# silverlight6/Ultrasound_Modeling

Hardware: AMD Instinct MI355X
Metric: segmentation training images/sec at 256x256 (higher is better)
Workload: dtype bf16

## Files before the change

### include/usseg.h

```cpp
#ifndef USSEG_H
#define USSEG_H

#include <stddef.h>
#include <stdint.h>

#ifdef __cplusplus
extern "C" {
#endif

typedef void* usseg_stream_t;

typedef enum UssegStatus {
  USSEG_OK = 0,
  USSEG_ERR_BAD_ARG = -1,
  USSEG_ERR_UNSUPPORTED = -2,
  USSEG_ERR_LAUNCH = -3
} UssegStatus;

typedef enum UssegAct { USSEG_ACT_NONE = 0, USSEG_ACT_LRELU = 1, USSEG_ACT_RELU = 2, USSEG_ACT_ELU = 3, USSEG_ACT_GELU = 4 } UssegAct;

enum {
  USSEG_OUT_F32 = 1,
  USSEG_ACCUMULATE = 2
};
// ... 49 lines not shown
int usseg_tconv2d_wgrad_mapped(const UssegConvDesc* d, const void* x, const void* dy, const UssegWgradDst* dst, float* ws,
                               int64_t ws_floats, usseg_stream_t stream);

typedef struct UssegWgradJob {
  UssegConvDesc desc;
  const void* x;
  const void* dy;
  float* dw;
  const UssegWgradDst* dst;
} UssegWgradJob;
int usseg_conv2d_wgrad_multi(int32_t njobs, const UssegWgradJob* jobs, float* ws, int64_t ws_floats, usseg_stream_t stream);

int usseg_defer_begin(usseg_stream_t stream, float* reduce_ws, int64_t reduce_floats, float* wgrad_ws, int64_t wgrad_floats);
int usseg_defer_flush(usseg_stream_t stream);
int usseg_defer_end(usseg_stream_t stream);

typedef struct UssegConvJob {
  UssegConvDesc desc;
  const void* x;
  const void* wp;
  const float* bias;
  const void* residual;
  int32_t ldr;
  int32_t reserved;
  void* y;
  const float* scale;
} UssegConvJob;
int usseg_conv2d_fwd_multi(int32_t njobs, const UssegConvJob* jobs, usseg_stream_t stream);
int usseg_conv2d_dgrad_multi(int32_t njobs, const UssegConvJob* jobs, usseg_stream_t stream);

// ... 377 lines not shown
```

### ultrasound_modeling_amd/_lib.py

```python
from __future__ import annotations

import ctypes as C
import os

import torch
from . import knobs

_HERE = os.path.dirname(os.path.abspath(__file__))
LIB_PATH = knobs.get("USSEG_LIB") or os.path.join(_HERE, "libusseg_hip.so")

c_i32, c_i64, c_f32, c_vp = C.c_int32, C.c_int64, C.c_float, C.c_void_p


class UssegError(RuntimeError):
    pass


class ConvDesc(C.Structure):
    _fields_ = [("B", c_i32), ("H", c_i32), ("W", c_i32), ("Cin", c_i32), ("Cout", c_i32), ("ldx", c_i32),
                ("ldy", c_i32), ("ksize", c_i32), ("dilation", c_i32), ("act", c_i32), ("alpha", c_f32),
                ("flags", c_i32)]


class ConvJob(C.Structure):
# ... 208 lines not shown
    "usseg_scale_f32": (C.c_int, [c_vp, c_i64, c_vp, c_f32, c_vp]),
    "usseg_sched_advance": (C.c_int, [c_vp, c_vp, c_vp, c_vp, c_f32, c_f32, c_vp]),
    "usseg_sumsq_sched_advance": (C.c_int, [c_vp, c_i64, c_vp, c_vp, c_vp, c_vp, c_vp, c_f32, c_f32, c_vp]),
    "usseg_adamw_step": (C.c_int, [c_vp, c_vp, c_vp, c_vp, c_i64, c_vp, c_f32, c_vp, c_vp, c_vp, c_f32, c_f32, c_f32, c_vp]),
    "usseg_gemm_nt_batched": (C.c_int, [P(GemmDesc), c_vp, c_vp, c_vp, c_vp]),
    "usseg_gemm_tn_batched": (C.c_int, [P(GemmDesc), c_vp, c_vp, c_vp, c_vp]),
    "usseg_flash_attn_fwd": (C.c_int, [P(FlashDesc), c_vp, c_vp, c_vp, c_vp, c_vp, c_vp, c_vp]),
    "usseg_flash_attn_bwd": (C.c_int, [P(FlashDesc), c_vp, c_vp, c_vp, c_vp, c_vp, c_vp, c_vp, c_vp, c_vp, c_vp, c_vp, c_vp]),
    "usseg_softmax_rows_fwd": (C.c_int, [c_vp, c_i64, c_i32, c_f32, c_vp, c_vp, c_vp]),
    "usseg_softmax_rows_bwd": (C.c_int, [c_vp, c_vp, c_i64, c_i32, c_f32, c_vp, c_vp]),
    "usseg_transpose_batched": (C.c_int, [c_vp, c_i32, c_i32, c_i32, c_i32, c_i32, c_i64, c_i64, c_vp, c_vp]),
    "usseg_cast_f32_to_bf16_batched": (C.c_int, [c_vp, c_i32, c_i32, c_i32, c_i32, c_vp, c_i32, c_i64, c_i64, c_vp]),
    "usseg_defer_begin": (C.c_int, [c_vp, c_vp, c_i64, c_vp, c_i64]),
    "usseg_defer_flush": (C.c_int, [c_vp]),
    "usseg_defer_end": (C.c_int, [c_vp]),
    "usseg_prof_enable": (C.c_int, [c_i32, c_i32]),
    "usseg_prof_read": (C.c_int, [c_i32, P(C.c_double), P(c_i64)]),
    "usseg_prof_disable": (C.c_int, []),
    "usseg_prep_cycle_stats": (C.c_int, [c_vp, c_i32, c_i32, c_i32, c_vp, c_vp, c_vp]),
    "usseg_prep_label": (C.c_int, [c_vp, c_i32, c_i32, c_vp, c_vp, c_i32, c_i32, c_i32, c_vp, c_vp, c_vp, c_vp]),
    "usseg_prep_label_thick": (C.c_int, [c_vp, c_i32, c_i32, c_vp, c_i32, c_i32, c_i32, c_vp, c_vp, c_vp]),
    "usseg_prep_assemble": (C.c_int, [c_vp, c_vp, c_i32, c_i32, c_i32, c_vp, c_i32, c_i32, c_i32, c_vp, c_vp, c_i32, c_vp, c_vp]),
    "usseg_select_ranks_f64": (C.c_int, [c_vp, c_i32, c_i64, P(c_i32), c_i32, c_vp, c_vp, c_vp]),
    "usseg_prep_aug_ws_doubles": (c_i64, [c_i32, c_i32, c_i32, c_i32, c_i32]),
    "usseg_prep_aug": (C.c_int, [P(PrepAugDesc), c_vp, c_vp, c_vp, c_vp, c_vp, c_i64, c_vp, c_vp, c_vp]),
    "usseg_cone_index": (C.c_int, [c_vp, c_vp, c_i32, c_i32, C.c_double, C.c_double, C.c_double, c_i32, c_i32, c_vp, c_vp]),
    "usseg_cone_range": (C.c_int, [c_vp, c_i32, c_i32, c_vp, c_vp, c_vp]),
    "usseg_cone_render": (C.c_int, [c_vp, c_i32, c_i32, c_i32, c_vp, c_vp, c_vp, c_vp, c_i32, c_i32, c_i32, P(C.c_double), c_vp, c_vp, c_vp,
                                    c_vp]),
}
# ... 26 lines not shown
```

### ultrasound_modeling_amd/csrc/common.h

```cpp
#pragma once
#include <hip/hip_runtime.h>
#include <stdint.h>
#include <stdio.h>
#include <stdlib.h>
#include "../../include/usseg.h"
#include "knobs.h"

typedef unsigned short bf16_t;
typedef __attribute__((ext_vector_type(8))) __bf16 bf16x8_t;
typedef __attribute__((ext_vector_type(4))) float f32x4_t;
typedef __attribute__((ext_vector_type(4))) short s16x4_t;

__device__ __forceinline__ float fdiv_rcp(int d) { return 0.5f * __builtin_amdgcn_rcpf((float)d); }
__device__ __forceinline__ int fdiv(int n, float r) {
  float x;
  asm("v_mul_f32_e32 %0, %1, %2" : "=v"(x) : "v"((float)(2 * n + 1)), "v"(r));
  return (int)x;
}
__device__ __forceinline__ void fdivmod(int n, int d, float r, int& q, int& rem) {
  q = fdiv(n, r);
  rem = n - __mul24(q, d);
}

__device__ __forceinline__ float fdiv_rcp1(int d) { return __builtin_amdgcn_rcpf((float)d); }
// ... 392 lines not shown
  UssegTapMask mask = {};
};
static inline WgHaloGeom wgrad_halo_geom(const UssegConvDesc& d, const void* x, const void* dy, float* out, const WgMap& map,
                                         const UssegTapMask& mask = {}) {
  WgHaloGeom g = {(const bf16_t*)x, (const bf16_t*)dy, out, map, d.B, d.H, d.W, d.dilation, d.Cin, d.Cout, d.ldx, d.ldy};
  g.mask = mask;
  return g;
}
int usseg_try_launch_wgrad_halo(const WgHaloGeom* g, int njobs, float* ws, int64_t ws_floats, hipStream_t s);
int conv2d_wgrad_impl(const UssegConvDesc* d, const void* x, const void* dy, float* dw, const UssegWgradDst* dst, float* ws, int64_t ws_floats,
                      const UssegTapMask& mask, usseg_stream_t stream);

float* usseg_defer_reduce_ws(hipStream_t s, float* caller_ws, int64_t need);
void usseg_defer_reduce_ws_n(hipStream_t s, float* caller_ws, const int64_t* need, int n, float** out);
float* usseg_defer_wgrad_ws(hipStream_t s, float* caller_ws, int64_t caller_floats, int64_t* avail);
void usseg_launch_wgrad_finish(const float* ws, int splits, int64_t slab_floats, float* out, const WgMap& map, int Ma, int Nb, hipStream_t s);

int usseg_try_launch_tconv_wgrad_halo(const bf16_t* x, const bf16_t* dy, const WgMap& map, int B, int H, int W, int Cin, int Cout, int ldx,
                                      int lddy, int k, float* ws, int64_t ws_floats, hipStream_t s);

static inline int64_t cdiv64(int64_t a, int64_t b) { return (a + b - 1) / b; }
```

### ultrasound_modeling_amd/csrc/defer.hip

```cpp
#include <vector>
#include "common.h"

struct RJob {
  const float* ws;
  float *d0, *d1, *d2;
  int32_t groups, nb, K, Cp, C, nblocks;
  float scale;
  int32_t overwrite;
};
struct RBatch {
  int32_t njobs, pad;
  int32_t start[60];
  RJob job[59];
};
static_assert(sizeof(RBatch) <= 4096, "RBatch must fit the kernel-argument segment");

__device__ __forceinline__ void reduce_finish_body(const RJob& q, int bx, int nbx) {
  __shared__ float s_part[16][17];
  const int total = q.groups * q.K * q.C;
  const int o = threadIdx.x & 15, sl = threadIdx.x >> 4;
  for (int base = bx * 16; base < total; base += nbx * 16) {
    const int i = base + o;
    float s = 0.f;
    int c = 0, k = 0, g = 0;
// ... 146 lines not shown
    RBatch b = {};
    int total = 0;
    while (i < c.rj.size() && b.njobs < 59 && !rjob_shares_dst(b, c.rj[i])) {
      b.job[b.njobs] = c.rj[i++];
      b.start[b.njobs] = total;
      total += b.job[b.njobs].nblocks;
      ++b.njobs;
    }
    b.start[b.njobs] = total;
    hipLaunchKernelGGL(reduce_finish_batched_kernel, dim3(total), dim3(256), 0, c.s, b);
  }
  c.rj.clear();
  c.rused = 0;
}
static void flush_wgrad(DeferCtx& c) {
  size_t i = 0;
  while (i < c.wj.size()) {
    WBatch b = {};
    int total = 0;
    while (i < c.wj.size() && b.njobs < 14 && !wjob_shares_dst(b, c.wj[i])) {
      b.job[b.njobs] = c.wj[i++];
      b.start[b.njobs] = total;
      total += b.job[b.njobs].gx;
      ++b.njobs;
    }
    b.start[b.njobs] = total;
    const int slot = usseg_prof_start(2, c.s);
    hipLaunchKernelGGL(wgrad_finish_batched_kernel, dim3(total), dim3(256), 0, c.s, b);
    usseg_prof_stop(2, slot, c.s);
  }
// ... 32 lines not shown
  if (c && c->rws && ws >= c->rws && ws < c->rws + c->rcap) {
    c->rj.push_back(q);
    return;
  }
  hipLaunchKernelGGL(reduce_finish_kernel, dim3(grid), dim3(256), 0, s, q);
}

float* usseg_defer_wgrad_ws(hipStream_t s, float* caller_ws, int64_t caller_floats, int64_t* avail) {
  DeferCtx* c = find_ctx(s);
  if (!c || !c->wws) { *avail = caller_floats; return caller_ws; }
  if (c->wcap - c->wused < c->wcap / 4 && !c->wj.empty()) flush_wgrad(*c);
  *avail = c->wcap - c->wused;
  return c->wws + c->wused;
}

void usseg_launch_wgrad_finish(const float* ws, int splits, int64_t slab_floats, float* out, const WgMap& map, int Ma, int Nb, hipStream_t s) {
  WJob q = {};
  q.ws = ws; q.out = out; q.n4 = slab_floats / 4; q.splits = splits; q.Ma = Ma; q.Nb = Nb; q.map = map;
  int sl_log2 = 2;
  while (sl_log2 < 6 && (q.n4 + (256 >> sl_log2) - 1) / (256 >> sl_log2) < 256 && splits >= (2 << (sl_log2 + 2))) sl_log2 += 2;
  const int O = 256 >> sl_log2;
  int gx = (int)((q.n4 + O - 1) / O);
  if (gx > 2048) gx = 2048;
  q.gx = gx; q.sl_log2 = sl_log2;
  DeferCtx* c = find_ctx(s);
  if (c && c->wws && ws >= c->wws && ws < c->wws + c->wcap) {
    c->wused = (ws - c->wws) + (((int64_t)splits * slab_floats + 63) & ~(int64_t)63);
    c->wj.push_back(q);
    return;
  }
  hipLaunchKernelGGL(wgrad_finish_kernel, dim3(gx), dim3(256), 0, s, q);
}

extern "C" int usseg_defer_begin(usseg_stream_t stream, float* reduce_ws, int64_t reduce_floats, float* wgrad_ws, int64_t wgrad_floats) {
  USSEG_CHECK_ARG((!reduce_ws || reduce_floats > 0) && (!wgrad_ws || wgrad_floats > 0), "defer_begin: bad workspace sizes");
  hipStream_t s = (hipStream_t)stream;
  DeferCtx* c = find_ctx(s);
  if (c) { flush_reduce(*c); flush_wgrad(*c); }
  else { g_ctx.push_back(DeferCtx()); c = &g_ctx.back(); c->s = s; }
  c->rws = reduce_ws; c->rcap = reduce_ws ? reduce_floats : 0; c->rused = 0;
  c->wws = wgrad_ws; c->wcap = wgrad_ws ? wgrad_floats : 0; c->wused = 0;
  return USSEG_OK;
// ... 18 lines not shown
```

### ultrasound_modeling_amd/csrc/knobs.h

```cpp
#pragma once
#include <stdint.h>
#include <stdlib.h>

#define USSEG_KNOBS(X)                                                                                                                  \
                                                                                                                      \
  X(K_BIG,                "USSEG_BIG",                INT,     1,     ONCE,     "0: conv_big and the streaming conv take no launch")        \
  X(K_BIG_PX,             "USSEG_BIG_PX",             INT,     0,     ONCE,     "conv_big: force the pixel tile (128 / 256; 0: planner)")   \
  X(K_BIG_NT,             "USSEG_BIG_NT",             INT,     0,     ONCE,     "conv_big: force the channel tile (1 / 2 / 4 x 16; 0: planner)") \
  X(K_BIG_MIN_WG,         "USSEG_BIG_MIN_WG",         INT,     128,   ONCE,     "conv_big: smallest launch it takes, in workgroups")        \
  X(K_BIG_WG_TILE,        "USSEG_BIG_WG_TILE",        INT,     512,   ONCE,     "conv_big: narrow the channel tile below this many workgroups") \
  X(K_BIG_MIN_CIN,        "USSEG_BIG_MIN_CIN",        INT,     33,    ONCE,     "conv_big: fewest input channels of a pass it takes")       \
  X(K_BIG_STAGES,         "USSEG_BIG_STAGES",         INT,     0,     ONCE,     "conv_big LDS stages: 0 by launch size, 1 / 2 forced")      \
  X(K_BIG_W8,             "USSEG_BIG_W8",             INT,     1,     PER_CALL, "256-pixel tile on eight waves: 0 never, 1 planner, 2 forced") \
  X(K_BIG_W8_MIN,         "USSEG_BIG_W8_MIN",         INT,     128,   ONCE,     "fewest workgroups left for the eight-wave tile")           \
  X(K_STREAM,             "USSEG_STREAM",             INT,     1,     ONCE,     "0: the streaming conv takes no launch")                    \
  X(K_STREAM_PX,          "USSEG_STREAM_PX",          INT,     0,     ONCE,     "streaming conv: force the pixel tile (128 / 256; 0: planner)") \
  X(K_STREAM_MIN_STEPS,   "USSEG_STREAM_MIN_STEPS",   INT,     1,     PER_CALL, "streaming conv: fewest K steps per workgroup it takes")    \
  X(K_STREAM_WGX,         "USSEG_STREAM_WGX",         INT,     0,     PER_CALL, "streaming conv: force grid.x (>= 8, rounded down to a multiple of 8)") \
  X(K_STREAM_OCC,         "USSEG_STREAM_OCC",         INT,     0,     ONCE,     "streaming conv: cap on workgroups per CU (0: by LDS)")     \
  X(K_STREAM_RES,         "USSEG_STREAM_RES",         INT,     1,     ONCE,     "0: passes with a residual do not stream")                  \
  X(K_STREAM_MULTI,       "USSEG_STREAM_MULTI",       INT,     1,     ONCE,     "0: multi-job launches do not stream")                      \
  X(K_STREAM_MERGE,       "USSEG_STREAM_MERGE",       INT,     1,     PER_CALL, "streaming jobs of one plan in one launch (0: a launch per job)") \
                                                                                                     \
  X(K_NO_HALO,            "USSEG_NO_HALO",            PRESENT, 0,     ONCE,     "the halo-tile conv and weight-gradient kernels take no launch") \
// ... 7 lines not shown
  X(K_IGEMM_DMA_BATCHED,  "USSEG_IGEMM_DMA_BATCHED",  INT,     1,     ONCE,     "0: batched GEMMs stay on the register-staged igemm")       \
  X(K_IGEMM_XCD,          "USSEG_IGEMM_XCD",          INT,     1,     ONCE,     "XCD-aware item order: 0 off, 1 activation-heavy launches, 2 all") \
  X(K_IGEMM_PERSIST,      "USSEG_IGEMM_PERSIST",      INT,     1,     ONCE,     "0: never the persistent LDS-DMA igemm")                    \
  X(K_IGEMM_STAGES8,      "USSEG_IGEMM_STAGES8",      INT,     4,     ONCE,     "ring depth of sparse long-K 128-channel launches (2: off, 3, 4)") \
  X(K_IGEMM_STAGES8_WG,   "USSEG_IGEMM_STAGES8_WG",   INT,     256,   ONCE,     "largest launch, in workgroups, that gets the deeper ring") \
                                                                                                         \
  X(K_WGRAD_DMA,          "USSEG_WGRAD_DMA",          INT,     1,     ONCE,     "0: never the LDS-DMA per-tap weight gradient / batched TN GEMM") \
  X(K_WGRAD_TM,           "USSEG_WGRAD_TM",           INT,     0,     ONCE,     "per-tap wgrad: force the tile (1: 64x64, 2: 128x128; 0: planner)") \
  X(K_WGD_TARGET,         "USSEG_WGD_TARGET",         INT,     512,   ONCE,     "per-tap wgrad: workgroups the split-K aims for")           \
  X(K_WGD_CAP,            "USSEG_WGD_CAP",            INT,     4,     ONCE,     "per-tap wgrad: slab traffic cap, in multiples of the operand bytes") \
  X(K_WG_QUANT,           "USSEG_WG_QUANT",           INT,     1,     ONCE,     "0: no wave-quantisation search of the split count (both wgrad kernels)") \
  X(K_WGRAD_DEBUG,        "USSEG_WGRAD_DEBUG",        PRESENT, 0,     ONCE,     "print every weight-gradient plan to stderr")               \
  X(K_WGRAD_POW2,         "USSEG_WGRAD_POW2",         INT,     1,     ONCE,     "0: no shift decode of power-of-two grids")                 \
  X(K_WGRAD_XCD,          "USSEG_WGRAD_XCD",          INT,     1,     ONCE,     "0: no XCD-aware item order in the per-tap wgrad")          \
  X(K_WG_TARGET,          "USSEG_WG_TARGET",          INT,     256,   ONCE,     "halo wgrad: workgroups the split-K aims for")              \
  X(K_SLAB_CAP,           "USSEG_SLAB_CAP",           INT,     2,     ONCE,     "halo wgrad: slab traffic cap, in multiples of the operand bytes") \
  X(K_WGHALO_XCD,         "USSEG_WGHALO_XCD",         INT,     1,     ONCE,     "0: no XCD-aware item order in the halo wgrad")             \
  X(K_WGRAD_PF,           "USSEG_WGRAD_PF",           INT,     1,     ONCE,     "0: halo wgrad without the register prefetch")              \
  X(K_WGRAD_8W,           "USSEG_WGRAD_8W",           INT,     1,     ONCE,     "0: the 64x64 halo wgrad tile on four waves, not eight")    \
  X(K_TCONV_HALO,         "USSEG_TCONV_HALO",         INT,     0,     PER_CALL, "1: transposed-conv wgrad as four parity-class halo jobs")  \
                                                                                                                      \
  X(K_CARD_BWD_G,         "USSEG_CARD_BWD_G",         INT,     0,     ONCE,     "fused cardinal backward: force the workgroup pairs (0: one resident wave)") \
  X(K_LN_TILE,            "USSEG_LN_TILE",            INT,     1,     ONCE,     "0: never the tile LayerNorm backward")                     \
  X(K_LN_PAIR,            "USSEG_LN_PAIR",            INT,     1,     ONCE,     "0: never the paired LayerNorm backward launch")            \
  X(K_LN_TILE_MIN,        "USSEG_LN_TILE_MIN",        INT,     32768, ONCE,     "fewest pixels for the tile / paired LayerNorm backward")   \
                                                                                     \
  X(K_FLASH_TILE,         "USSEG_FLASH_TILE",         INT,     -1,    ONCE,     "fused attention tiling 0 / 1 / 2 (-1: by problem size)")   \
  X(K_WINATTN_MFMA,       "USSEG_WINATTN_MFMA",       INT,     1,     ONCE,     "0: window attention without the MFMA kernels")             \
  X(K_LOSS_PPT,           "USSEG_LOSS_PPT",           INT,     4,     ONCE,     "softmax + loss kernel: pixels per thread")

// ... 26 lines not shown
```

### ultrasound_modeling_amd/csrc/wgrad_halo.hip

```cpp
#include "common.h"

struct WgHaloParams {
  const bf16_t* x;
  const bf16_t* dy;
  float* out;
  float* ws;
  int32_t B, H, W, d, Hl, Wl, PH, PW, NV;
  int32_t tiles_x, tiles_per_v, npatches, ngroups, groups_per_block;
  int32_t ldx, lddy, Ma, Nb, ntiles_n;
  int32_t mask_ch;
  uint16_t tapmask[4];
  int32_t xvd, xvH, xvW, xva, xvb;
  int32_t yvd, yvH, yvW, yva, yvb;
};

struct WgHaloMulti {
  WgHaloParams job[4];
  int32_t xcd_remap;
};

template <int WVM, int WM, int WN, bool PF, int NTG, bool MASKED>
__global__ __launch_bounds__(256 * NTG, NTG == 1 ? 2 : 1) void wgrad_halo_kernel(const WgHaloMulti P) {
  constexpr int NTHR = 256 * NTG, TPG = NTG == 1 ? 9 : 5;
  int bx = blockIdx.x, by = blockIdx.y, bz = blockIdx.z;
  if (P.xcd_remap) {
    const int gx = gridDim.x, gy = gridDim.y, gz = gridDim.z, total = gx * gy * gz;
    const int L = bx + gx * (by + gy * bz);
    const int c = L & 7, q = total >> 3, r = total & 7;
    const int item = c * q + (c < r ? c : r) + (L >> 3);
    const int u = __builtin_amdgcn_readfirstlane(fdiv(item, fdiv_rcp(gy)));
    by = item - u * gy;
    bx = __builtin_amdgcn_readfirstlane(fdiv(u, fdiv_rcp(gz)));
    bz = u - bx * gz;
  }
  const WgHaloParams& p = P.job[bz];
  constexpr int MAXHP = 288;
  constexpr int WVN = 4 / WVM;
  constexpr int BMc = 16 * WM * WVM, BNc = 16 * WN * WVN;
  constexpr int XS = BMc + 16, YS = BNc == 16 ? 48 : BNc + 16;
  constexpr int XCH = BMc / 8, YCH = BNc / 8;
  constexpr int X_IT = (MAXHP * XCH + NTHR - 1) / NTHR, Y_IT = (128 * YCH + NTHR - 1) / NTHR;
  __shared__ __attribute__((aligned(16))) bf16_t lds_x[MAXHP * XS];
  __shared__ __attribute__((aligned(16))) bf16_t lds_y[128 * YS];
  constexpr int TB = NTHR / 8;
  __shared__ __attribute__((aligned(16))) int s_tab[TB][8][8];

  const int tid = threadIdx.x, lane = tid & 63, wv = (tid >> 6) & 3, tg = tid >> 8;
  const int t0 = tg * TPG;
  const int HW2 = p.PW + 2, HPP = (p.PH + 2) * HW2, NHP = p.NV * HPP;
  const int rps = 16 / p.PW, spp = (p.PH * p.PW) >> 4;
// ... 248 lines not shown
        if (m >= p.Ma || n >= p.Nb) continue;
        float* q = dst + ((int64_t)t * p.Ma + m) * p.Nb + n;
        if (p.ws && vec_ok && n + 3 < p.Nb) {
          *reinterpret_cast<float4*>(q) = make_float4(acc[tt][i][j][0], acc[tt][i][j][1], acc[tt][i][j][2], acc[tt][i][j][3]);
        } else {
#pragma unroll
          for (int r = 0; r < 4; ++r)
            if (n + r < p.Nb) {
              if (p.ws) q[r] = acc[tt][i][j][r];
              else atomicAdd(q + r, acc[tt][i][j][r]);
            }
        }
      }
}

int usseg_try_launch_wgrad_halo(const WgHaloGeom* gm, int njobs, float* ws, int64_t ws_floats, hipStream_t s) {
  const int disabled = knob<K_NO_HALO>();
  if (disabled || njobs < 1 || njobs > 4) return 0;
  WgHaloMulti P;
  const int Ma = gm[0].Ma, Nb = gm[0].Nb;
  auto shape_of = [](int ma, int nb) { return (ma <= 32 && nb <= 32) ? 1 : (nb <= 16 ? 2 : (nb <= 32 ? 3 : 0)); };
  auto tiles_of = [&](int ma, int nb) {
    const int sh = shape_of(ma, nb), bm = sh == 1 ? 32 : 64, bn = sh == 0 ? 64 : (sh == 2 ? 16 : 32);
    return ((ma + bm - 1) / bm) * ((nb + bn - 1) / bn);
  };
  int64_t slab_max = 0, slab_sum = 0;
  for (int j = 0; j < njobs; ++j) {
    const WgHaloGeom& q = gm[j];
    if (q.B != gm[0].B || q.H != gm[0].H || q.W != gm[0].W) return 0;
    if (shape_of(q.Ma, q.Nb) != shape_of(Ma, Nb) || tiles_of(q.Ma, q.Nb) != tiles_of(Ma, Nb)) return 0;
    if ((q.Ma != Ma || q.Nb != Nb) && (q.mask.group_ch || q.tconv_cls >= 0)) return 0;
    slab_sum += (int64_t)9 * q.Ma * q.Nb;
    if ((int64_t)9 * q.Ma * q.Nb > slab_max) slab_max = (int64_t)9 * q.Ma * q.Nb;
    const int d = q.d;
// ... 32 lines not shown
  if (ws) ws = usseg_defer_wgrad_ws(s, ws, ws_floats, &ws_floats);
  int shape = 0;
  if (Ma <= 32 && Nb <= 32) shape = 1;
  else if (Nb <= 16) shape = 2;
  else if (Nb <= 32) shape = 3;
  const int bm = shape == 1 ? 32 : 64, bn = shape == 0 ? 64 : (shape == 2 ? 16 : 32);
  const int tm = (Ma + bm - 1) / bm;
  const int ntn = (Nb + bn - 1) / bn;
  const int tiles = tm * ntn;
  const int ngroups = P.job[0].ngroups;
  const int64_t slab = slab_max;
  int64_t in_bytes = 0;
  for (int j = 0; j < njobs; ++j) in_bytes += (int64_t)gm[j].B * gm[j].H * gm[j].W * (gm[j].Ma + gm[j].Nb) * 2;
  in_bytes /= njobs;
  const int64_t slab_bytes = slab * 4;
  const int wg_target = knob<K_WG_TARGET>();
  int splits = (wg_target + tiles * njobs - 1) / (tiles * njobs);
  int max_splits = (ngroups + 1) / 2;
  const int slab_cap = knob<K_SLAB_CAP>();
  const int64_t traffic_cap = slab_cap * in_bytes / slab_bytes < 4 ? 4 : slab_cap * in_bytes / slab_bytes;
  if (max_splits > traffic_cap) max_splits = (int)traffic_cap;
  if (!ws) max_splits = (ngroups + 15) / 16;
  else if ((int64_t)max_splits * slab_sum > ws_floats) max_splits = (int)(ws_floats / slab_sum);
  if (splits > max_splits) splits = max_splits;
  if (splits < 1) splits = 1;
  {
    const int quant = knob<K_WG_QUANT>();
    if (quant && max_splits > 1) {
      const int slots = 256 * (shape == 0 ? 1 : 2);
      const int64_t tj = (int64_t)tiles * njobs;
      int best = splits;
// ... 19 lines not shown
    int64_t off = 0;
    for (int j = 0; j < njobs; ++j) {
      P.job[j].ntiles_n = (gm[j].Nb + bn - 1) / bn;
      P.job[j].groups_per_block = gpb;
      P.job[j].ws = use_ws ? ws + off : nullptr;
      off += (int64_t)splits * 9 * gm[j].Ma * gm[j].Nb;
    }
  }
  const UssegTapMask& qm = gm[0].mask;
  const bool masked = qm.group_ch != 0 || gm[0].tconv_cls >= 0;
  if (qm.group_ch) {
    if (njobs != 1 || qm.group_ch % bn) return 0;
    P.job[0].mask_ch = qm.group_ch;
    for (int c = 0; c < 4; ++c) P.job[0].tapmask[c] = qm.mask[c];
  }
  const dim3 grid(splits, tiles, njobs);
  const int xcd_env = knob<K_WGHALO_XCD>();
  P.xcd_remap = xcd_env && tiles * njobs > 1 && (int64_t)splits * tiles * njobs < (1ll << 20);
  const int dbg = knob<K_WGRAD_DEBUG>();
  if (dbg) fprintf(stderr, "[wgrad_halo] B %d H %d W %d d %d Ma %d Nb %d jobs %d shape %d tiles %d ngroups %d splits %d gpb %d max_splits %d traffic_cap %lld slab_MB %.2f in_MB %.2f\n",
                   gm[0].B, gm[0].H, gm[0].W, gm[0].d, Ma, Nb, njobs, shape, tiles, ngroups, splits, gpb, max_splits, (long long)traffic_cap, slab_bytes / 1e6, in_bytes / 1e6);
  const int slot = usseg_prof_start(2, s);
  const int pf = knob<K_WGRAD_PF>();
  if (shape == 1) {
    if (pf) { if (masked) hipLaunchKernelGGL((wgrad_halo_kernel<2, 1, 1, true, 1, true>), grid, dim3(256), 0, s, P); else hipLaunchKernelGGL((wgrad_halo_kernel<2, 1, 1, true, 1, false>), grid, dim3(256), 0, s, P); }
    else { if (masked) hipLaunchKernelGGL((wgrad_halo_kernel<2, 1, 1, false, 1, true>), grid, dim3(256), 0, s, P); else hipLaunchKernelGGL((wgrad_halo_kernel<2, 1, 1, false, 1, false>), grid, dim3(256), 0, s, P); }
  } else if (shape == 2) {
    if (pf) { if (masked) hipLaunchKernelGGL((wgrad_halo_kernel<4, 1, 1, true, 1, true>), grid, dim3(256), 0, s, P); else hipLaunchKernelGGL((wgrad_halo_kernel<4, 1, 1, true, 1, false>), grid, dim3(256), 0, s, P); }
    else { if (masked) hipLaunchKernelGGL((wgrad_halo_kernel<4, 1, 1, false, 1, true>), grid, dim3(256), 0, s, P); else hipLaunchKernelGGL((wgrad_halo_kernel<4, 1, 1, false, 1, false>), grid, dim3(256), 0, s, P); }
  } else if (shape == 3) {
    if (pf) { if (masked) hipLaunchKernelGGL((wgrad_halo_kernel<4, 1, 2, true, 1, true>), grid, dim3(256), 0, s, P); else hipLaunchKernelGGL((wgrad_halo_kernel<4, 1, 2, true, 1, false>), grid, dim3(256), 0, s, P); }
    else { if (masked) hipLaunchKernelGGL((wgrad_halo_kernel<4, 1, 2, false, 1, true>), grid, dim3(256), 0, s, P); else hipLaunchKernelGGL((wgrad_halo_kernel<4, 1, 2, false, 1, false>), grid, dim3(256), 0, s, P); }
  } else {
    const int tg8 = knob<K_WGRAD_8W>();
    if (tg8) { if (masked) hipLaunchKernelGGL((wgrad_halo_kernel<2, 2, 2, true, 2, true>), grid, dim3(512), 0, s, P); else hipLaunchKernelGGL((wgrad_halo_kernel<2, 2, 2, true, 2, false>), grid, dim3(512), 0, s, P); }
    else { if (masked) hipLaunchKernelGGL((wgrad_halo_kernel<2, 2, 2, false, 1, true>), grid, dim3(256), 0, s, P); else hipLaunchKernelGGL((wgrad_halo_kernel<2, 2, 2, false, 1, false>), grid, dim3(256), 0, s, P); }
  }
  if (use_ws)
    for (int j = 0; j < njobs; ++j) usseg_launch_wgrad_finish(P.job[j].ws, splits, (int64_t)9 * gm[j].Ma * gm[j].Nb, gm[j].out, gm[j].map, gm[j].Ma, gm[j].Nb, s);
  usseg_prof_stop(2, slot, s);
  return 1;
}

int usseg_try_launch_tconv_wgrad_halo(const bf16_t* x, const bf16_t* dy, const WgMap& map, int B, int H, int W, int Cin, int Cout, int ldx,
                                      int lddy, int k, float* ws, int64_t ws_floats, hipStream_t s) {
  const int enabled = knob<K_TCONV_HALO>();
  if (!enabled || map.nblocks < 1 || (k != 3 && k != 4)) return 0;
  const int pad = k == 4 ? 1 : 0;
  WgHaloGeom g[4];
  for (int c = 0; c < 4; ++c) {
    const int a = c >> 1, b = c & 1;
    uint32_t mask = 0;
    for (int th = 0; th < 3; ++th)
      for (int tw = 0; tw < 3; ++tw) {
        const int kh = a + pad - 2 + 2 * th, kw = b + pad - 2 + 2 * tw;
// ... 17 lines not shown
```

### ultrasound_modeling_amd/knobs.py

```python
from __future__ import annotations

import os

KNOBS = {
    "USSEG_LIB":                ("str",    None,  "path of a diagnostic build of the same sources to load instead of the in-tree library"),
    "USSEG_SIDE_STREAM":        ("flag",   0,     "weight gradients fork to a side stream per launch inside an overlap region"),
    "USSEG_DEFER":              ("flag",   1,     "defer the finishing reductions to the end of the region (0: finish after each producer)"),
    "USSEG_LAZY_WGRAD":         ("flag",   1,     "lazy weight gradients: queued and run on the side stream beside the backward-data chain"),
    "USSEG_FUSE_LN_RES":        ("flag",   1,     "LayerNorm backward + residual add in one pass (transformer blocks)"),
    "USSEG_ENC_LAZY":           ("optint", None,  "bit mask of the ResNest stages whose weight gradients are lazy (unset: 12, or 0 in front of a ViT)"),
    "USSEG_FOLD_BN":            ("flag",   1,     "inference BatchNorm folded into the producing conv's packed weights"),
    "USSEG_FUSED_CARDINAL":     ("flag",   1,     "cardinal group + shortcut of a stage as one launch"),
    "USSEG_FUSED_CARDINAL_BWD": ("flag",   1,     "its backward chain + the shortcut norm's backward as one launch"),
    "USSEG_CARD_BWD_MAX_PX":    ("int",    32768, "most pixels of a stage for the fused cardinal backward"),
    "USSEG_LN_PAIR":            ("flag",   1,     "shortcut norm backward + conv2_bn backward of the large stages in one launch"),
    "USSEG_FUSED_STEM_BWD":     ("flag",   1,     "stem backward-data fused with the norm / activation backward in front"),
    "USSEG_STEM_WGRAD_MERGE":   ("flag",   1,     "the stem's three weight gradients in one multi-job launch"),
    "USSEG_FUSED_STEM":         ("flag",   1,     "the stem (three convs, two norms, pool) as one launch"),
    "USSEG_MERGED_DGRAD":       ("flag",   1,     "one backward-data GEMM for a stage's grouped 1x1 and shortcut 1x1"),
    "USSEG_FUSED_DGRAD":        ("flag",   1,     "the DecoderBlock's four branch backward-data passes as one launch"),
    "USSEG_BRANCH4":            ("flag",   1,     "the DecoderBlock's 1x1 branch as a fourth job of the dilated branches' launch"),
    "USSEG_QUAD_UP":            ("flag",   0,     "the decoder's transposed convs in quad (parity-class) form"),
    "USSEG_QUAD_HEAD":          ("flag",   1,     "the <= 4-class head's transposed conv in quad form (read at construction)"),
    "USSEG_QUAD_TCONV":         ("flag",   0,     "Arch A's inner transposed convs in quad form (read at construction)"),
# ... 19 lines not shown
```

### ultrasound_modeling_amd/ops.py

```python
from __future__ import annotations

import contextlib
import ctypes as C
import math
import os
from typing import Optional, Tuple

import torch

from . import _lib as L
from . import knobs
from ._lib import (ACCUMULATE, ACT_ELU, ACT_GELU, ACT_LRELU, ACT_NONE, ACT_RELU, OUT_F32, CardinalDesc, ConvDesc, GemmDesc, LossDesc, NormDesc,
                   SplitAttnDesc, SplitAttnGrads, SplitAttnParams)

BF16 = torch.bfloat16
ACC_FLOATS = 2050


def roundup(a: int, b: int) -> int:
    return (a + b - 1) // b * b


def _stream() -> int:
    return torch.cuda.current_stream().cuda_stream
# ... 94 lines not shown
    if _Side.stream is None:
        _Side.stream = torch.cuda.Stream()
    main = torch.cuda.current_stream()
    ev = torch.cuda.Event()
    ev.record(main)
    _Side.stream.wait_event(ev)
    _Side.keep.extend(keep)
    _Side.dirty = True
    with torch.cuda.stream(_Side.stream):
        _defer_begin()
        yield


_LAZY = knobs.get("USSEG_LAZY_WGRAD")
_lazy_q = None


@contextlib.contextmanager
def lazy_wgrads():
    global _lazy_q
    if not _LAZY or _Side.depth == 0 or _lazy_q is not None:
        yield
        return
    _lazy_q = []
    try:
        yield
    finally:
        q, _lazy_q = _lazy_q, None
        if q:
            enabled, _Side.enabled = _Side.enabled, True
            try:
                with side_stream(*[t for _, keep in q for t in keep]):
                    for fn, _ in q:
                        fn()
            finally:
                _Side.enabled = enabled


def wgrad_later(fn, *keep):
    if _lazy_q is not None:
        _lazy_q.append((fn, keep))
        return
    with side_stream(*keep):
        fn()


def side_join():
    if _Side.dirty:
        with torch.cuda.stream(_Side.stream):
            _defer_end()
        ev = torch.cuda.Event()
        ev.record(_Side.stream)
        torch.cuda.current_stream().wait_event(ev)
        _Side.dirty = False
    _Side.keep.clear()


def _ws_key(device):
    on_side = _Side.stream is not None and torch.cuda.current_stream() == _Side.stream
# ... 1158 lines not shown
```

Baseline: 5599.

## Batch queued halo weight-gradient jobs into one table-driven launch per tile shape

The halo wgrad kernel now takes a flat job table of up to 16 jobs with per-job start offsets instead of a 3D grid over at most 4 jobs. Inside a lazy weight-gradient block, halo wgrad launches are queued per stream and emitted together, one launch per shape and mask variant, sorted by groups per block. The aim is fewer kernel launches and better GPU fill when many small wgrads run side by side. A separate split-K workgroup target knob applies to coscheduled jobs but defaults to the old value. The change also adds flush and ordering logic: pending jobs are launched before deferred reductions and when an output pointer repeats, and the workspace high-water mark now only moves up.

```diff
diff --git a/include/usseg.h b/include/usseg.h
--- a/include/usseg.h
+++ b/include/usseg.h
@@ -87,6 +87,10 @@
 int usseg_defer_begin(usseg_stream_t stream, float* reduce_ws, int64_t reduce_floats, float* wgrad_ws, int64_t wgrad_floats);
 int usseg_defer_flush(usseg_stream_t stream);
 int usseg_defer_end(usseg_stream_t stream);
+
+int usseg_wgrad_batch_begin(usseg_stream_t stream);
+int usseg_wgrad_batch_end(usseg_stream_t stream);
+int usseg_wgrad_coscheduled(int32_t on);
 
 typedef struct UssegConvJob {
   UssegConvDesc desc;
diff --git a/ultrasound_modeling_amd/_lib.py b/ultrasound_modeling_amd/_lib.py
--- a/ultrasound_modeling_amd/_lib.py
+++ b/ultrasound_modeling_amd/_lib.py
@@ -246,6 +246,9 @@
     "usseg_defer_begin": (C.c_int, [c_vp, c_vp, c_i64, c_vp, c_i64]),
     "usseg_defer_flush": (C.c_int, [c_vp]),
     "usseg_defer_end": (C.c_int, [c_vp]),
+    "usseg_wgrad_batch_begin": (C.c_int, [c_vp]),
+    "usseg_wgrad_batch_end": (C.c_int, [c_vp]),
+    "usseg_wgrad_coscheduled": (C.c_int, [c_i32]),
     "usseg_prof_enable": (C.c_int, [c_i32, c_i32]),
     "usseg_prof_read": (C.c_int, [c_i32, P(C.c_double), P(c_i64)]),
     "usseg_prof_disable": (C.c_int, []),
diff --git a/ultrasound_modeling_amd/csrc/common.h b/ultrasound_modeling_amd/csrc/common.h
--- a/ultrasound_modeling_amd/csrc/common.h
+++ b/ultrasound_modeling_amd/csrc/common.h
@@ -430,6 +430,8 @@
 float* usseg_defer_reduce_ws(hipStream_t s, float* caller_ws, int64_t need);
 void usseg_defer_reduce_ws_n(hipStream_t s, float* caller_ws, const int64_t* need, int n, float** out);
 float* usseg_defer_wgrad_ws(hipStream_t s, float* caller_ws, int64_t caller_floats, int64_t* avail);
+bool usseg_defer_owns_wgrad_ws(hipStream_t s, const float* ws);
+void usseg_wgrad_batch_launch_pending(hipStream_t s);
 void usseg_launch_wgrad_finish(const float* ws, int splits, int64_t slab_floats, float* out, const WgMap& map, int Ma, int Nb, hipStream_t s);
 
 int usseg_try_launch_tconv_wgrad_halo(const bf16_t* x, const bf16_t* dy, const WgMap& map, int B, int H, int W, int Cin, int Cout, int ldx,
diff --git a/ultrasound_modeling_amd/csrc/defer.hip b/ultrasound_modeling_amd/csrc/defer.hip
--- a/ultrasound_modeling_amd/csrc/defer.hip
+++ b/ultrasound_modeling_amd/csrc/defer.hip
@@ -184,6 +184,7 @@
   c.rused = 0;
 }
 static void flush_wgrad(DeferCtx& c) {
+  usseg_wgrad_batch_launch_pending(c.s);
   size_t i = 0;
   while (i < c.wj.size()) {
     WBatch b = {};
@@ -246,6 +247,11 @@
   return c->wws + c->wused;
 }
 
+bool usseg_defer_owns_wgrad_ws(hipStream_t s, const float* ws) {
+  DeferCtx* c = find_ctx(s);
+  return c && c->wws && ws >= c->wws && ws < c->wws + c->wcap;
+}
+
 void usseg_launch_wgrad_finish(const float* ws, int splits, int64_t slab_floats, float* out, const WgMap& map, int Ma, int Nb, hipStream_t s) {
   WJob q = {};
   q.ws = ws; q.out = out; q.n4 = slab_floats / 4; q.splits = splits; q.Ma = Ma; q.Nb = Nb; q.map = map;
@@ -257,7 +263,8 @@
   q.gx = gx; q.sl_log2 = sl_log2;
   DeferCtx* c = find_ctx(s);
   if (c && c->wws && ws >= c->wws && ws < c->wws + c->wcap) {
-    c->wused = (ws - c->wws) + (((int64_t)splits * slab_floats + 63) & ~(int64_t)63);
+    const int64_t end = (ws - c->wws) + (((int64_t)splits * slab_floats + 63) & ~(int64_t)63);
+    if (end > c->wused) c->wused = end;
     c->wj.push_back(q);
     return;
   }
diff --git a/ultrasound_modeling_amd/csrc/knobs.h b/ultrasound_modeling_amd/csrc/knobs.h
--- a/ultrasound_modeling_amd/csrc/knobs.h
+++ b/ultrasound_modeling_amd/csrc/knobs.h
@@ -45,6 +45,7 @@
   X(K_WGRAD_POW2,         "USSEG_WGRAD_POW2",         INT,     1,     ONCE,     "0: no shift decode of power-of-two grids")                 \
   X(K_WGRAD_XCD,          "USSEG_WGRAD_XCD",          INT,     1,     ONCE,     "0: no XCD-aware item order in the per-tap wgrad")          \
   X(K_WG_TARGET,          "USSEG_WG_TARGET",          INT,     256,   ONCE,     "halo wgrad: workgroups the split-K aims for")              \
+  X(K_WG_TARGET_BATCHED,  "USSEG_WG_TARGET_BATCHED",  INT,     256,   ONCE,     "halo wgrad: the target of jobs issued together (usseg_wgrad_coscheduled)") \
   X(K_SLAB_CAP,           "USSEG_SLAB_CAP",           INT,     2,     ONCE,     "halo wgrad: slab traffic cap, in multiples of the operand bytes") \
   X(K_WGHALO_XCD,         "USSEG_WGHALO_XCD",         INT,     1,     ONCE,     "0: no XCD-aware item order in the halo wgrad")             \
   X(K_WGRAD_PF,           "USSEG_WGRAD_PF",           INT,     1,     ONCE,     "0: halo wgrad without the register prefetch")              \
diff --git a/ultrasound_modeling_amd/csrc/wgrad_halo.hip b/ultrasound_modeling_amd/csrc/wgrad_halo.hip
--- a/ultrasound_modeling_amd/csrc/wgrad_halo.hip
+++ b/ultrasound_modeling_amd/csrc/wgrad_halo.hip
@@ -1,3 +1,5 @@
+#include <algorithm>
+#include <vector>
 #include "common.h"
 
 struct WgHaloParams {
@@ -12,28 +14,38 @@
   uint16_t tapmask[4];
   int32_t xvd, xvH, xvW, xva, xvb;
   int32_t yvd, yvH, yvW, yva, yvb;
+  int32_t tiles, splits;
+  int32_t xcd_remap, pad;
 };
 
-struct WgHaloMulti {
-  WgHaloParams job[4];
-  int32_t xcd_remap;
+#define WGH_MAX_JOBS 16
+struct WgHaloTable {
+  int32_t njobs, pad;
+  int32_t start[WGH_MAX_JOBS];
+  WgHaloParams job[WGH_MAX_JOBS];
 };
+static_assert(sizeof(WgHaloTable) <= 4096, "WgHaloTable must fit the kernel-argument segment");
 
 template <int WVM, int WM, int WN, bool PF, int NTG, bool MASKED>
-__global__ __launch_bounds__(256 * NTG, NTG == 1 ? 2 : 1) void wgrad_halo_kernel(const WgHaloMulti P) {
+__global__ __launch_bounds__(256 * NTG, NTG == 1 ? 2 : 1) void wgrad_halo_kernel(const WgHaloTable P) {
   constexpr int NTHR = 256 * NTG, TPG = NTG == 1 ? 9 : 5;
-  int bx = blockIdx.x, by = blockIdx.y, bz = blockIdx.z;
-  if (P.xcd_remap) {
-    const int gx = gridDim.x, gy = gridDim.y, gz = gridDim.z, total = gx * gy * gz;
-    const int L = bx + gx * (by + gy * bz);
+  int bz = 0;
+#pragma unroll
+  for (int j = 1; j < WGH_MAX_JOBS; ++j) bz += (j < P.njobs && (int)blockIdx.x >= P.start[j]) ? 1 : 0;
+  const WgHaloParams& p = P.job[bz];
+  const int L = (int)blockIdx.x - P.start[bz];
+  const int total = p.splits * p.tiles;
+  if (L >= total) return;
+  int bx, by;
+  if (p.xcd_remap) {
     const int c = L & 7, q = total >> 3, r = total & 7;
     const int item = c * q + (c < r ? c : r) + (L >> 3);
-    const int u = __builtin_amdgcn_readfirstlane(fdiv(item, fdiv_rcp(gy)));
-    by = item - u * gy;
-    bx = __builtin_amdgcn_readfirstlane(fdiv(u, fdiv_rcp(gz)));
-    bz = u - bx * gz;
-  }
-  const WgHaloParams& p = P.job[bz];
+    bx = __builtin_amdgcn_readfirstlane(fdiv(item, fdiv_rcp(p.tiles)));
+    by = item - bx * p.tiles;
+  } else {
+    by = __builtin_amdgcn_readfirstlane(fdiv(L, fdiv_rcp(p.splits)));
+    bx = L - by * p.splits;
+  }
   constexpr int MAXHP = 288;
   constexpr int WVN = 4 / WVM;
   constexpr int BMc = 16 * WM * WVM, BNc = 16 * WN * WVN;
@@ -312,10 +324,96 @@
       }
 }
 
+static void launch_table(const WgHaloTable& P, int total, int shape, bool masked, hipStream_t s) {
+  const dim3 grid(total);
+  const int slot = usseg_prof_start(2, s);
+  const int pf = knob<K_WGRAD_PF>();
+  if (shape == 1) {
+    if (pf) { if (masked) hipLaunchKernelGGL((wgrad_halo_kernel<2, 1, 1, true, 1, true>), grid, dim3(256), 0, s, P); else hipLaunchKernelGGL((wgrad_halo_kernel<2, 1, 1, true, 1, false>), grid, dim3(256), 0, s, P); }
+    else { if (masked) hipLaunchKernelGGL((wgrad_halo_kernel<2, 1, 1, false, 1, true>), grid, dim3(256), 0, s, P); else hipLaunchKernelGGL((wgrad_halo_kernel<2, 1, 1, false, 1, false>), grid, dim3(256), 0, s, P); }
+  } else if (shape == 2) {
+    if (pf) { if (masked) hipLaunchKernelGGL((wgrad_halo_kernel<4, 1, 1, true, 1, true>), grid, dim3(256), 0, s, P); else hipLaunchKernelGGL((wgrad_halo_kernel<4, 1, 1, true, 1, false>), grid, dim3(256), 0, s, P); }
+    else { if (masked) hipLaunchKernelGGL((wgrad_halo_kernel<4, 1, 1, false, 1, true>), grid, dim3(256), 0, s, P); else hipLaunchKernelGGL((wgrad_halo_kernel<4, 1, 1, false, 1, false>), grid, dim3(256), 0, s, P); }
+  } else if (shape == 3) {
+    if (pf) { if (masked) hipLaunchKernelGGL((wgrad_halo_kernel<4, 1, 2, true, 1, true>), grid, dim3(256), 0, s, P); else hipLaunchKernelGGL((wgrad_halo_kernel<4, 1, 2, true, 1, false>), grid, dim3(256), 0, s, P); }
+    else { if (masked) hipLaunchKernelGGL((wgrad_halo_kernel<4, 1, 2, false, 1, true>), grid, dim3(256), 0, s, P); else hipLaunchKernelGGL((wgrad_halo_kernel<4, 1, 2, false, 1, false>), grid, dim3(256), 0, s, P); }
+  } else {
+    const int tg8 = knob<K_WGRAD_8W>();
+    if (tg8) { if (masked) hipLaunchKernelGGL((wgrad_halo_kernel<2, 2, 2, true, 2, true>), grid, dim3(512), 0, s, P); else hipLaunchKernelGGL((wgrad_halo_kernel<2, 2, 2, true, 2, false>), grid, dim3(512), 0, s, P); }
+    else { if (masked) hipLaunchKernelGGL((wgrad_halo_kernel<2, 2, 2, false, 1, true>), grid, dim3(256), 0, s, P); else hipLaunchKernelGGL((wgrad_halo_kernel<2, 2, 2, false, 1, false>), grid, dim3(256), 0, s, P); }
+  }
+  usseg_prof_stop(2, slot, s);
+}
+
+struct WgQueued { WgHaloParams p; int shape; bool masked; };
+struct WgBatchCtx { hipStream_t s; int depth; std::vector<WgQueued> q; };
+static thread_local std::vector<WgBatchCtx> g_batch;
+static thread_local int g_cosched = 0;
+
+static WgBatchCtx* find_batch(hipStream_t s) {
+  for (auto& c : g_batch)
+    if (c.s == s) return &c;
+  return nullptr;
+}
+
+static void launch_pending(WgBatchCtx& c) {
+  std::vector<WgQueued> q;
+  q.swap(c.q);
+  std::vector<char> done(q.size(), 0);
+  for (size_t i = 0; i < q.size(); ++i) {
+    if (done[i]) continue;
+    std::vector<const WgQueued*> grp;
+    for (size_t k = i; k < q.size(); ++k)
+      if (!done[k] && q[k].shape == q[i].shape && q[k].masked == q[i].masked) { grp.push_back(&q[k]); done[k] = 1; }
+    for (size_t c0 = 0; c0 < grp.size(); c0 += WGH_MAX_JOBS) {
+      const size_t n = grp.size() - c0 < WGH_MAX_JOBS ? grp.size() - c0 : WGH_MAX_JOBS;
+      std::stable_sort(grp.begin() + c0, grp.begin() + c0 + n, [](const WgQueued* a, const WgQueued* b) { return a->p.groups_per_block > b->p.groups_per_block; });
+      WgHaloTable T = {};
+      T.njobs = (int)n;
+      int total = 0;
+      for (size_t j = 0; j < n; ++j) {
+        T.job[j] = grp[c0 + j]->p;
+        T.start[j] = total;
+        const int wgs = T.job[j].splits * T.job[j].tiles;
+        total += j + 1 < n ? (wgs + 7) & ~7 : wgs;
+      }
+      launch_table(T, total, q[i].shape, q[i].masked, c.s);
+    }
+  }
+}
+
+void usseg_wgrad_batch_launch_pending(hipStream_t s) {
+  WgBatchCtx* c = find_batch(s);
+  if (c && !c->q.empty()) launch_pending(*c);
+}
+
+extern "C" int usseg_wgrad_batch_begin(usseg_stream_t stream) {
+  hipStream_t s = (hipStream_t)stream;
+  WgBatchCtx* c = find_batch(s);
+  if (c) { ++c->depth; return USSEG_OK; }
+  g_batch.push_back(WgBatchCtx{s, 1, {}});
+  return USSEG_OK;
+}
+extern "C" int usseg_wgrad_batch_end(usseg_stream_t stream) {
+  hipStream_t s = (hipStream_t)stream;
+  for (size_t i = 0; i < g_batch.size(); ++i)
+    if (g_batch[i].s == s) {
+      if (--g_batch[i].depth > 0) return USSEG_OK;
+      if (!g_batch[i].q.empty()) launch_pending(g_batch[i]);
+      g_batch.erase(g_batch.begin() + i);
+      break;
+    }
+  return usseg_check_launch("wgrad_batch_end");
+}
+extern "C" int usseg_wgrad_coscheduled(int32_t on) {
+  g_cosched = on != 0;
+  return USSEG_OK;
+}
+
 int usseg_try_launch_wgrad_halo(const WgHaloGeom* gm, int njobs, float* ws, int64_t ws_floats, hipStream_t s) {
   const int disabled = knob<K_NO_HALO>();
   if (disabled || njobs < 1 || njobs > 4) return 0;
-  WgHaloMulti P;
+  struct { WgHaloParams job[4]; } P;
   const int Ma = gm[0].Ma, Nb = gm[0].Nb;
   auto shape_of = [](int ma, int nb) { return (ma <= 32 && nb <= 32) ? 1 : (nb <= 16 ? 2 : (nb <= 32 ? 3 : 0)); };
   auto tiles_of = [&](int ma, int nb) {
@@ -378,7 +476,7 @@
   for (int j = 0; j < njobs; ++j) in_bytes += (int64_t)gm[j].B * gm[j].H * gm[j].W * (gm[j].Ma + gm[j].Nb) * 2;
   in_bytes /= njobs;
   const int64_t slab_bytes = slab * 4;
-  const int wg_target = knob<K_WG_TARGET>();
+  const int wg_target = g_cosched ? knob<K_WG_TARGET_BATCHED>() : knob<K_WG_TARGET>();
   int splits = (wg_target + tiles * njobs - 1) / (tiles * njobs);
   int max_splits = (ngroups + 1) / 2;
   const int slab_cap = knob<K_SLAB_CAP>();
@@ -428,31 +526,41 @@
     P.job[0].mask_ch = qm.group_ch;
     for (int c = 0; c < 4; ++c) P.job[0].tapmask[c] = qm.mask[c];
   }
-  const dim3 grid(splits, tiles, njobs);
   const int xcd_env = knob<K_WGHALO_XCD>();
-  P.xcd_remap = xcd_env && tiles * njobs > 1 && (int64_t)splits * tiles * njobs < (1ll << 20);
   const int dbg = knob<K_WGRAD_DEBUG>();
   if (dbg) fprintf(stderr, "[wgrad_halo] B %d H %d W %d d %d Ma %d Nb %d jobs %d shape %d tiles %d ngroups %d splits %d gpb %d max_splits %d traffic_cap %lld slab_MB %.2f in_MB %.2f\n",
                    gm[0].B, gm[0].H, gm[0].W, gm[0].d, Ma, Nb, njobs, shape, tiles, ngroups, splits, gpb, max_splits, (long long)traffic_cap, slab_bytes / 1e6, in_bytes / 1e6);
-  const int slot = usseg_prof_start(2, s);
-  const int pf = knob<K_WGRAD_PF>();
-  if (shape == 1) {
-    if (pf) { if (masked) hipLaunchKernelGGL((wgrad_halo_kernel<2, 1, 1, true, 1, true>), grid, dim3(256), 0, s, P); else hipLaunchKernelGGL((wgrad_halo_kernel<2, 1, 1, true, 1, false>), grid, dim3(256), 0, s, P); }
-    else { if (masked) hipLaunchKernelGGL((wgrad_halo_kernel<2, 1, 1, false, 1, true>), grid, dim3(256), 0, s, P); else hipLaunchKernelGGL((wgrad_halo_kernel<2, 1, 1, false, 1, false>), grid, dim3(256), 0, s, P); }
-  } else if (shape == 2) {
-    if (pf) { if (masked) hipLaunchKernelGGL((wgrad_halo_kernel<4, 1, 1, true, 1, true>), grid, dim3(256), 0, s, P); else hipLaunchKernelGGL((wgrad_halo_kernel<4, 1, 1, true, 1, false>), grid, dim3(256), 0, s, P); }
-    else { if (masked) hipLaunchKernelGGL((wgrad_halo_kernel<4, 1, 1, false, 1, true>), grid, dim3(256), 0, s, P); else hipLaunchKernelGGL((wgrad_halo_kernel<4, 1, 1, false, 1, false>), grid, dim3(256), 0, s, P); }
-  } else if (shape == 3) {
-    if (pf) { if (masked) hipLaunchKernelGGL((wgrad_halo_kernel<4, 1, 2, true, 1, true>), grid, dim3(256), 0, s, P); else hipLaunchKernelGGL((wgrad_halo_kernel<4, 1, 2, true, 1, false>), grid, dim3(256), 0, s, P); }
-    else { if (masked) hipLaunchKernelGGL((wgrad_halo_kernel<4, 1, 2, false, 1, true>), grid, dim3(256), 0, s, P); else hipLaunchKernelGGL((wgrad_halo_kernel<4, 1, 2, false, 1, false>), grid, dim3(256), 0, s, P); }
+  for (int j = 0; j < njobs; ++j) {
+    P.job[j].tiles = tiles;
+    P.job[j].splits = splits;
+    P.job[j].xcd_remap = xcd_env && tiles > 1 && (int64_t)splits * tiles < (1ll << 20);
+  }
+  WgBatchCtx* bc = find_batch(s);
+  const bool queue = bc && (!use_ws || usseg_defer_owns_wgrad_ws(s, ws));
+  if (queue && !use_ws)
+    for (const WgQueued& q : bc->q) {
+      bool same = false;
+      for (int j = 0; j < njobs; ++j) same = same || q.p.out == gm[j].out;
+      if (same) { launch_pending(*bc); break; }
+    }
+  if (queue) {
+    for (int j = 0; j < njobs; ++j) bc->q.push_back({P.job[j], shape, masked});
   } else {
-    const int tg8 = knob<K_WGRAD_8W>();
-    if (tg8) { if (masked) hipLaunchKernelGGL((wgrad_halo_kernel<2, 2, 2, true, 2, true>), grid, dim3(512), 0, s, P); else hipLaunchKernelGGL((wgrad_halo_kernel<2, 2, 2, true, 2, false>), grid, dim3(512), 0, s, P); }
-    else { if (masked) hipLaunchKernelGGL((wgrad_halo_kernel<2, 2, 2, false, 1, true>), grid, dim3(256), 0, s, P); else hipLaunchKernelGGL((wgrad_halo_kernel<2, 2, 2, false, 1, false>), grid, dim3(256), 0, s, P); }
-  }
-  if (use_ws)
+    WgHaloTable T = {};
+    T.njobs = njobs;
+    int total = 0;
+    for (int j = 0; j < njobs; ++j) {
+      T.job[j] = P.job[j];
+      T.start[j] = total;
+      total += j + 1 < njobs ? (splits * tiles + 7) & ~7 : splits * tiles;
+    }
+    launch_table(T, total, shape, masked, s);
+  }
+  if (use_ws) {
+    const int slot = queue ? -1 : usseg_prof_start(2, s);
     for (int j = 0; j < njobs; ++j) usseg_launch_wgrad_finish(P.job[j].ws, splits, (int64_t)9 * gm[j].Ma * gm[j].Nb, gm[j].out, gm[j].map, gm[j].Ma, gm[j].Nb, s);
-  usseg_prof_stop(2, slot, s);
+    if (!queue) usseg_prof_stop(2, slot, s);
+  }
   return 1;
 }
 
diff --git a/ultrasound_modeling_amd/knobs.py b/ultrasound_modeling_amd/knobs.py
--- a/ultrasound_modeling_amd/knobs.py
+++ b/ultrasound_modeling_amd/knobs.py
@@ -7,6 +7,7 @@
     "USSEG_SIDE_STREAM":        ("flag",   0,     "weight gradients fork to a side stream per launch inside an overlap region"),
     "USSEG_DEFER":              ("flag",   1,     "defer the finishing reductions to the end of the region (0: finish after each producer)"),
     "USSEG_LAZY_WGRAD":         ("flag",   1,     "lazy weight gradients: queued and run on the side stream beside the backward-data chain"),
+    "USSEG_WGRAD_BATCH":        ("flag",   1,     "the halo weight gradients of a lazy block queued and launched together, one launch per tile shape"),
     "USSEG_FUSE_LN_RES":        ("flag",   1,     "LayerNorm backward + residual add in one pass (transformer blocks)"),
     "USSEG_ENC_LAZY":           ("optint", None,  "bit mask of the ResNest stages whose weight gradients are lazy (unset: 12, or 0 in front of a ViT)"),
     "USSEG_FOLD_BN":            ("flag",   1,     "inference BatchNorm folded into the producing conv's packed weights"),
diff --git a/ultrasound_modeling_amd/ops.py b/ultrasound_modeling_amd/ops.py
--- a/ultrasound_modeling_amd/ops.py
+++ b/ultrasound_modeling_amd/ops.py
@@ -132,25 +132,54 @@
 
 _LAZY = knobs.get("USSEG_LAZY_WGRAD")
 _lazy_q = None
+_WGRAD_BATCH = knobs.get("USSEG_WGRAD_BATCH")
+_lazy_depth = 0
+
+
+@contextlib.contextmanager
+def _coscheduled():
+    lib = L.load()
+    lib.usseg_wgrad_coscheduled(1)
+    try:
+        yield
+    finally:
+        lib.usseg_wgrad_coscheduled(0)
 
 
 @contextlib.contextmanager
 def lazy_wgrads():
-    global _lazy_q
-    if not _LAZY or _Side.depth == 0 or _lazy_q is not None:
+    global _lazy_q, _lazy_depth
+    if _Side.depth == 0:
         yield
+        return
+    _lazy_depth += 1
+    if not _LAZY or _lazy_q is not None:
+        try:
+            yield
+        finally:
+            _lazy_depth -= 1
         return
     _lazy_q = []
     try:
         yield
     finally:
+        _lazy_depth -= 1
         q, _lazy_q = _lazy_q, None
         if q:
             enabled, _Side.enabled = _Side.enabled, True
             try:
-                with side_stream(*[t for _, keep in q for t in keep]):
-                    for fn, _ in q:
-                        fn()
+                with side_stream(*[t for _, keep in q for t in keep]), _coscheduled():
+                    if _WGRAD_BATCH:
+                        h = _stream()
+                        L.check(L.load().usseg_wgrad_batch_begin(h), "wgrad_batch_begin")
+                        try:
+                            for fn, _ in q:
+                                fn()
+                        finally:
+                            L.check(L.load().usseg_wgrad_batch_end(h), "wgrad_batch_end")
+                    else:
+                        for fn, _ in q:
+                            fn()
             finally:
                 _Side.enabled = enabled
 
@@ -160,7 +189,11 @@
         _lazy_q.append((fn, keep))
         return
     with side_stream(*keep):
-        fn()
+        if _lazy_depth > 0:
+            with _coscheduled():
+                fn()
+        else:
+            fn()
 
 
 def side_join():
```

After: 5480. 2.1% lower.
